# careylab/LocoMouse_cpp

Measured on AMD Instinct MI355X. Metric: frames/sec whole-node + achieved HBM GB/s; 1024×256 gray, 6 templates, higher is better.
Workload: dtype f32

## Files before the change

### include/locomouse_hip.h

```cpp
#ifndef LOCOMOUSE_HIP_H
#define LOCOMOUSE_HIP_H

#include <stddef.h>
#include <stdint.h>

#ifdef __cplusplus
extern "C" {
#endif

#define LM_ABI_VERSION 6
#define LM_N_PAWS 4
#define LM_N_TAIL_POINTS 15
#define LM_N_LISTS 4
#define LM_N_FEATURES 2

typedef enum {
  LM_OK = 0,
  LM_ERR_INVALID_ARGUMENT = 1,
  LM_ERR_RUNTIME = 2,
  LM_ERR_HIP = 3
} lm_status;

typedef struct {
  int32_t x, y, width, height;
// ... 145 lines not shown

lm_status lm_ctx_set_debug(lm_ctx* ctx, int32_t flags);

lm_status lm_debug_scores(lm_ctx* ctx, int32_t f, int32_t det, float* out, int32_t rows, int32_t cols);

lm_status lm_debug_tail_mask(lm_ctx* ctx, int32_t f, uint8_t* out, int32_t rows, int32_t cols);

int32_t lm_debug_kernel_times(lm_ctx* ctx, const char** names, double* ms, int32_t cap);

int32_t lm_debug_kernel_spans(lm_ctx* ctx, const char** names, double* t0, double* t1, int32_t cap);

lm_status lm_debug_corr_work(const lm_ctx* ctx, int32_t* out);

lm_status lm_debug_tail_work(lm_ctx* ctx, int32_t* out);

lm_status lm_debug_tail_tiles(lm_ctx* ctx, int32_t f, int32_t view, uint8_t* out, int32_t rows, int32_t cols);

lm_status lm_debug_point_work(lm_ctx* ctx, int32_t* out);

lm_status lm_debug_point_tiles(lm_ctx* ctx, int32_t f, int32_t det, uint8_t* out, int32_t rows, int32_t cols);

int32_t lm_debug_dark_tile_width(void);
int32_t lm_debug_dark_tile_height(void);

int32_t lm_debug_batch_slots(const lm_ctx* ctx);


#define LM_BB_FIRSTLAST_AS_EXECUTED 0
#define LM_BB_FIRSTLAST_INTEGER 1

// ... 53 lines not shown
```

### locomouse_cpp_amd/csrc/lm_device.h

```cpp
#ifndef LM_DEVICE_H
#define LM_DEVICE_H

#include <stdint.h>

#if defined(__HIPCC__)
#define LM_HD __host__ __device__
#else
#define LM_HD
#endif

#define LM_C 5
#define LM_R 3
#define LM_TW (16 * LM_C)
#define LM_TH (16 * LM_R)
#define LM_JC 4
#ifndef LM_FW
#define LM_FW 40
#endif
#ifndef LM_FH
#define LM_FH 4
#endif
static_assert((LM_FW == 40 || LM_FW == 80) && (LM_FH == 4 || LM_FH == 8), "dark-tile grid");
#define LM_RW_NQX (LM_TW / LM_FW)
#define LM_RW_NQY (16 / LM_FH)
// ... 47 lines not shown
  int32_t tail_w, tail_hb, tail_hs;
  int32_t tail_cap, tail_ntc;
  int32_t tail_nw, tail_bm_words;
  int32_t connectivity;
  int32_t fl_tx[2], fl_ty[2], fl_off[2], fl_slot;
  int32_t tl_stride;
  int32_t tt_tx[2], tt_ty[2], tt_off[2], tt_slot;
  int32_t tt_stride;
  int64_t pt_plane;
  int32_t tb_skip[LM_NDET], tb_off[LM_NDET], tb_rng[LM_NDET], tb_lds[2];
  double tb_bias[LM_NDET];
  int32_t tbw_br[2], tbw_nband[2], tbw_blo[2], tbw_nbk[2], tbw_rows[2], tbw_v[2], tbw_al[2], tbw_work[2], tbw_lds[2];
  int32_t tbw_use[LM_NDET], tbw_pn[LM_NDET], tbw_win[LM_NDET], tbw_wsz[LM_NDET], tbw_ent[LM_NDET];
  uint32_t tbw_inv[LM_NDET];
  int32_t tbr_on[LM_NDET], tbr_ng[LM_NDET], tbr_off[LM_NDET];
  int32_t fl_my[2], fl_mx[2], fl_oh[2], fl_ow[2];
  int32_t ing_b0[2], ing_nb[2], ing_threads;
  int32_t list_cap[LM_NLIST];
  int64_t list_off[LM_NLIST];
  int64_t keys_per_slot;
  double side_bottom_min_overlap;
  double alpha_vel_bottom, pairwise_occluded_cost;
  int32_t max_displacement_bottom, ong_spacing_bottom;
  int32_t ong_nx, ong_ny;
  double ong_br_x, ong_br_y;
  int32_t bb_bottom_w, bb_bottom_h;
  int32_t spre_b_w, spre_b_h, spre_t_w, spre_t_h;
  int32_t match_b[LM_NFEAT][4];
  int32_t match_s[LM_NFEAT][4];
  int32_t size_b[LM_NFEAT][2];
// ... 108 lines not shown
```

### locomouse_cpp_amd/csrc/lm_kernels.hip

```cpp
#include <hip/hip_runtime.h>
#include <stdint.h>

#include <type_traits>
#include <utility>

#include "lm_device.h"
#include "lm_introsort.h"

#include "lm_dev_common.h"
#include "lm_tail_bound.h"
#include "lm_tile_plan.h"



__global__ __launch_bounds__(LM_MM_THREADS) void k_minmax(const uint8_t* const* __restrict__ frame_ptr,
                                                          const uint8_t* __restrict__ bkg, int npix, int s0,
                                                          unsigned* __restrict__ mm) {
  const int slot = s0 + blockIdx.y;
  const lm_gu8* __restrict__ F = as_global(frame_ptr[slot]);
  const int nvec = npix >> 4;
  const int per = (nvec + LM_MM_SPLIT - 1) / LM_MM_SPLIT;
  const int v0 = blockIdx.x * per, v1 = min(nvec, v0 + per);
  const lm_gu4* F4 = reinterpret_cast<const lm_gu4*>(F);
  const uint4* B4 = reinterpret_cast<const uint4*>(bkg);
// ... 626 lines not shown
  if (m == 0ull) return 0;
  const int rank = (int)__builtin_amdgcn_mbcnt_hi((unsigned)(m >> 32), __builtin_amdgcn_mbcnt_lo((unsigned)m, 0u));
  int base = 0;
  if (p && rank == 0) base = atomicAdd(ctr, (int)__popcll(m));
  return __shfl(base, __ffsll((long long)m) - 1) + rank;
}
#ifndef LM_TBW_WPE
#define LM_TBW_WPE 8
#endif
#define TBW_SEL(a) (k == 0 ? a[0] : k == 1 ? a[1] : a[2])
template <bool ROWS>
__global__ __launch_bounds__(LM_TB_THREADS) __attribute__((amdgpu_waves_per_eu(LM_TBW_WPE, 8))) void k_tile_bound(
    const LmConst* __restrict__ Kp, const uint32_t* __restrict__ rng, int64_t rng_slot, int s0, int nslot,
    const double* __restrict__ tbc, const uint8_t* __restrict__ bright, uint8_t* __restrict__ tail_flags,
    int32_t* __restrict__ tt_cnt, uint32_t* __restrict__ tt_list, uint8_t* __restrict__ pt_flags,
    int32_t* __restrict__ pt_cnt, uint32_t* __restrict__ pt_list) {
  const LmConst& K = *Kp;
  extern __shared__ __attribute__((aligned(16))) uint8_t tbw_lds[];
  __shared__ int s_n[3], s_b[3], s_m[3], s_base[3], s_nw;
  const int v = (int)blockIdx.y < K.tbw_nband[0] ? 0 : 1;
  const int band = (int)blockIdx.y - (v ? K.tbw_nband[0] : 0);
  const int slot = s0 + (int)blockIdx.x;
  const int T = (int)blockDim.x, tid = (int)threadIdx.x;
  if (tid < 3) {
    s_n[tid] = 0;
    s_b[tid] = 0;
    s_m[tid] = 0;
  }
  if (tid == 0) s_nw = 0;
  bool on[3], use[3], refine[3], tail[3];
  int t0[3], nt[3], ohb[3], ftx[3], tbase[3];
// ... 207 lines not shown
    constexpr int WV = 64;
    const int c1 = (nr3[0] * LM_TB_NBX + WV - 1) / WV, c2 = c1 + (nr3[1] * LM_TB_NBX + WV - 1) / WV,
              c3 = c2 + (nr3[2] * LM_TB_NBX + WV - 1) / WV;
    const uint32_t rcx = lm_rcp(LM_TB_NBX);
    for (int ch = __builtin_amdgcn_readfirstlane(tid / WV); ch < c3; ch += T / WV) {
      const int k = ch < c1 ? 0 : ch < c2 ? 1 : 2;
      const int d = 3 * v + k;
      const LmDet& D = K.det[d];
      const int n = TBW_SEL(nr3), fx = TBW_SEL(ftx), tk0 = TBW_SEL(t0), ohk = TBW_SEL(ohb);
      const int e = (ch - (k == 0 ? 0 : k == 1 ? c1 : c2)) * WV + (tid & (WV - 1));
      const int mb = k == 0 ? 0 : k == 1 ? nr3[0] : nr3[0] + nr3[1];
      const uint32_t* ent = reinterpret_cast<const uint32_t*>(tbw_lds + K.tbw_ent[d]);
      const int kh = D.kh, ng = K.tbr_ng[d], nc = lm_tbr_chunks(ng);
      const double* __restrict__ C = tbc + K.tbr_off[d];
      const double bias = K.tb_bias[d];
      const int yb = D.in_y + LM_FH * tk0 - y_lo;
      const int bl0 = lm_tbr_block0(D.in_x, 0) - K.tbw_blo[v];
      const int bendl = lm_tbr_block_end(D.in_x, D.ow, D.kw, K.ext_w[v] / LM_TB_BLK) - K.tbw_blo[v];
      const int nbx = (D.ow + LM_TB_BLK - 1) / LM_TB_BLK;
      if (e >= n * LM_TB_NBX) continue;
      const int t = lm_div(e, rcx);
      const int tile = (int)(ent[t] & 0xFFFFu);
      const int ty = lm_div(tile, K.tbw_inv[d]), tx = tile - ty * fx;
      const int xb = tx * LM_TB_NBX + (e - t * LM_TB_NBX);
      if (xb >= nbx) continue;
      const int tyb = ty - tk0;
      const int nr = min(LM_TB_H, ohk - LM_TB_H * tyb);
      const int row0 = yb + LM_TB_H * tyb, ba0 = bl0 + xb;
      auto level_v = [&](auto rows) {
        const uint32_t* pw = V + row0 * nw + (ba0 >> 1);
        const uint16_t* alone = AL + k * als + row0;
        const bool clipped = ba0 + ng == bendl;
        const int jl = (ng - 1) % LM_TBR_GC;
        uint32_t w0, w1, w2, x0 = 0u, x1 = 0u;
        unsigned qn, q = 0u;
        bool lastc = false;
        auto fetch = [&]() {
          w0 = pw[0];
          w1 = pw[1];
          w2 = pw[2];
          qn = *alone;
        };
        fetch();
        if constexpr (decltype(rows)::value > 0) {
          constexpr int NG = decltype(rows)::value;
          return lm_tbr_sum_rows_n<NG>(kh, C, bias, [&](int i, int g, unsigned& M, unsigned& m) {
                   if (g == 0) {
                     lm_tbr_quad_align(w0, w1, w2, ba0, x0, x1);
                     q = qn;
                     pw += nw;
                     alone += 1;
                     fetch();
                   }
                   lm_tbr_quad_get(x0, x1, g, g == NG - 1 && clipped, q, M, m);
                 }) < 0.0;
        }
        return lm_tbr_sum_negative(kh, ng, C, bias, [&](int i, int g, unsigned& M, unsigned& m) {
          if (g % LM_TBR_GC == 0) {
            const int c = g / LM_TBR_GC;
            lm_tbr_quad_align(w0, w1, w2, ba0, x0, x1);
            q = qn;
            lastc = c == nc - 1;
            pw += lastc ? nw - 2 * (nc - 1) : 2;
            alone += lastc ? 1 : 0;
            fetch();
          }
          lm_tbr_quad_get(x0, x1, g % LM_TBR_GC, lastc && clipped && g % LM_TBR_GC == jl, q, M, m);
        });
      };
      auto level_b = [&](int rs, int nn) {
        return lm_tbr_sum_negative(kh, ng, C, bias, [&](int i, int g, unsigned& M, unsigned& m) {
          const uint16_t* row = B16 + (row0 + rs + i) * nbk;
          M = 0u;
          m = 255u;
          for (int r = 0; r < nn; ++r, row += nbk) {
            unsigned a, b;
            lm_tbr_pair_range(nullptr, row, ba0 + g, bendl, a, b);
            M = max(M, a);
            m = min(m, b);
          }
        });
      };
      using std::integral_constant;
      bool proven;
      if constexpr (!ROWS) {
        proven = nr == LM_TB_H && level_v(integral_constant<int, 0>{});
      } else {
        proven = false;
        if (nr != LM_TB_H) {
        } else if (nc != 1) proven = level_v(integral_constant<int, 0>{});
        else if (ng == 4) proven = level_v(integral_constant<int, 4>{});
        else if (ng == 3) proven = level_v(integral_constant<int, 3>{});
        else if (ng == 2) proven = level_v(integral_constant<int, 2>{});
        else proven = level_v(integral_constant<int, 1>{});
      }
      if (!proven && !(LM_TB_RH == LM_TB_H && nr == LM_TB_H)) {
        if (LM_TB_RH == LM_TB_H) {
          proven = level_b(0, nr);
        } else {
          proven = true;
          for (int r = 0; r < nr && proven; ++r) proven = level_b(r, 1);
        }
      }
      if (!proven) mark[mb + t] = 1u;
    }
    __syncthreads();
    constexpr int CR = LM_TBW_CR;
    for (int g0 = 0; g0 < nref; g0 += CR * T) {
      uint32_t en[CR];
// ... 1848 lines not shown
```

### locomouse_cpp_amd/csrc/lm_runtime.hip

```cpp
#include <hip/hip_runtime.h>

#include <algorithm>
#include <array>
#include <cmath>
#include <cstdio>
#include <cstring>
#include <map>
#include <numeric>
#include <atomic>
#include <deque>
#include <memory>
#include <mutex>
#include <stdexcept>
#include <string>
#include <thread>
#include <vector>

#include "locomouse_hip.h"
#include "lm_host.h"
#include "lm_kernels.hip"

namespace {

constexpr size_t kCorrLdsBudget = 64 * 1024;
// ... 153 lines not shown
  } corr_plan[2];
  DevBuf<uint8_t> bkg, adj;
  DevBuf<int32_t> cal;
  DevBuf<float> weights;
  DevBuf<_Float16> weights16;
  DevBuf<LmConst> dK;
  size_t tail_lds = 0;
  bool tail_big = false;
  int64_t tail_ws_slot = 0;
  bool kprof_on = false;
  bool dark_on = true;
  bool tailskip_on = true;
  bool pointskip_on = true;
  bool tb_ref = false;
  bool tb_refine = true;
  bool corr_dir_on = true;
  size_t tb_lds = 0;
  size_t tbw_lds = 0;
  bool tbw_row_loop = false;
  DevBuf<double> tb_const;
  std::vector<std::unique_ptr<Lane>> lanes;
  DevBuf<uint8_t> handoff;
  std::vector<std::unique_ptr<HostBuf<uint8_t>>> packs;
  std::vector<char> pack_busy;
  int take_pack(size_t cap) {
    size_t i = 0;
    while (i < packs.size() && pack_busy[i]) ++i;
    if (i == packs.size()) {
      packs.emplace_back(new HostBuf<uint8_t>());
      pack_busy.push_back(0);
    }
    if (packs[i]->n < cap) packs[i]->alloc(cap);
    pack_busy[i] = 1;
    return (int)i;
  }
// ... 101 lines not shown
        (f16_nch(dets[d]->cols) > LM_F16_MAX_NCH || f16_lds_bytes(f16_nch(dets[d]->cols), dets[d]->rows) > kF16LdsMax))
      throw std::invalid_argument(std::string(names[d]) + ": detector too large for the f16 correlation (LM_CORR_F16).");
  }
  if (su->corr_precision != LM_CORR_FP32 && su->corr_precision != LM_CORR_F16)
    throw std::invalid_argument("corr_precision must be LM_CORR_FP32 or LM_CORR_F16.");
}

LmTileSwitches read_switches(lm_ctx* c, const lm_setup* su) {
  auto flag = [](const char* name, bool dflt) {
    const char* v = getenv(name);
    return v ? atoi(v) != 0 : dflt;
  };
  c->kprof_on = flag("LM_KPROF", false);
  c->dark_on = flag("LM_CORR_DARK", true);
  c->tb_refine = flag("LM_TILE_REFINE", true);
  c->tb_ref = flag("LM_TILE_BOUND_REF", false);
  c->corr_dir_on = flag("LM_CORR_DIR", true);
  LmTileSwitches sw;
  sw.tailskip = flag("LM_CORR_TAILSKIP", true);
  sw.pointskip = flag("LM_CORR_POINTSKIP", true);
  sw.refine = c->tb_refine;
  sw.f16 = su->corr_precision == LM_CORR_F16;
  sw.dark = c->dark_on;
  return sw;
}

lm_geometry make_geometry(const lm_setup* su, const lm_params* P, const lm_model* M) {
  const int NR = su->calib_rows, NC = su->calib_cols;
  const lm_rect ub = P->bounding_box_bottom, us = P->bounding_box_side;
  lm_geometry g;
  std::memset(&g, 0, sizeof(g));
  g.n_rows = NR;
  g.n_cols = NC;
  const int mts_c = std::max(M->paw_side.cols, M->snout_side.cols), mts_r = std::max(M->paw_side.rows, M->snout_side.rows);
  const int mtb_c = std::max(M->paw_bottom.cols, M->snout_bottom.cols), mtb_r = std::max(M->paw_bottom.rows, M->snout_bottom.rows);
  g.spre_t_w = ceil_half(mts_c - 1);
// ... 371 lines not shown
  const int64_t nc = (int64_t)su->calib_rows * su->calib_cols;
  hipStream_t cs = nullptr;
  HIPCHK(hipStreamCreateWithFlags(&cs, hipStreamNonBlocking));
  struct StreamGuard {
    hipStream_t s;
    ~StreamGuard() { (void)hipStreamDestroy(s); }
  } cs_guard{cs};
  c->bkg.alloc(nv);
  COPY_SYNC(c->bkg.p, su->background, nv, hipMemcpyHostToDevice, cs);
  c->cal.alloc(nc);
  COPY_SYNC(c->cal.p, su->ind_warp_mapping, nc * sizeof(int32_t), hipMemcpyHostToDevice, cs);
  c->weights.alloc(wts.size());
  COPY_SYNC(c->weights.p, wts.data(), wts.size() * sizeof(float), hipMemcpyHostToDevice, cs);
  c->tb_const.alloc(tbc.size());
  COPY_SYNC(c->tb_const.p, tbc.data(), tbc.size() * sizeof(double), hipMemcpyHostToDevice, cs);
  if (!w16.empty()) {
    c->weights16.alloc(w16.size());
    COPY_SYNC(c->weights16.p, w16.data(), w16.size() * sizeof(_Float16), hipMemcpyHostToDevice, cs);
  }
  c->adj.alloc(256);
  COPY_SYNC(c->adj.p, adj, 256, hipMemcpyHostToDevice, cs);
  c->dK.alloc(1);
  COPY_SYNC(c->dK.p, &c->K, sizeof(LmConst), hipMemcpyHostToDevice, cs);
  c->fstride = (nv + 255) / 256 * 256;
  HIPCHK(hipFuncSetAttribute((const void*)k_tail<false>, hipFuncAttributeMaxDynamicSharedMemorySize, (int)c->tail_lds));
  HIPCHK(hipFuncSetAttribute((const void*)k_tile_bound_ref, hipFuncAttributeMaxDynamicSharedMemorySize, (int)c->tb_lds));
  HIPCHK(hipFuncSetAttribute((const void*)k_tile_bound<false>, hipFuncAttributeMaxDynamicSharedMemorySize, (int)c->tbw_lds));
  HIPCHK(hipFuncSetAttribute((const void*)k_tile_bound<true>, hipFuncAttributeMaxDynamicSharedMemorySize, (int)c->tbw_lds));
  for (const auto& P : c->corr_plan)
    for (size_t g = 0; g < P.groups.size(); ++g)
// ... 409 lines not shown
    k_ingest<<<dim3((unsigned)(K.ing_nb[0] + K.ing_nb[1]), (unsigned)((nproc + LM_INGEST_FB - 1) / LM_INGEST_FB)),
               K.ing_threads, 0, st>>>(dK, L.frame_ptr.p, c->bkg.p, c->cal.p, L.luts.p, L.slots.p, s_proc0, n + 1, L.ext.p,
                                        c->ext_slot_bytes, reinterpret_cast<unsigned*>(L.tailbin.p), L.smap.p, L.sbkg.p,
                                        L.skey.p, dk.flags, dk.cnt, dk.list, L.rng.p, kpi);
    T.end();
    if (dk.tail_cnt || dk.pt_cnt) {
      T.begin("k_tile_bound");
      if (c->tb_ref)
        k_tile_bound_ref<<<dim3((unsigned)nproc, 2), LM_TB_THREADS, c->tb_lds, st>>>(
            dK, L.ext.p, c->ext_slot_bytes, s_proc0, c->tb_const.p, dk.flags, dk.tail_flags, dk.tail_cnt, dk.tail_list,
            dk.pt_flags, dk.pt_cnt, dk.pt_list);
      else
        (c->tbw_row_loop ? k_tile_bound<true> : k_tile_bound<false>)
            <<<dim3((unsigned)nproc, (unsigned)(K.tbw_nband[0] + K.tbw_nband[1])), LM_TB_THREADS, c->tbw_lds, st>>>(
                dK, L.rng.p, c->ext_slot_bytes / LM_INGEST_VEC, s_proc0, nproc, c->tb_const.p, dk.flags, dk.tail_flags,
                dk.tail_cnt, dk.tail_list, dk.pt_flags, dk.pt_cnt, dk.pt_list);
      T.end();
    }
    const lm_ctx::CorrPlan& CP = c->corr_plan[P.plan];
    if (c->corr_dir_on && std::find(CP.ring.begin(), CP.ring.end(), (char)1) != CP.ring.end()) {
      std::vector<LmDetGroup> groups;
      for (const auto& grp : CP.groups) groups.push_back(grp.second);
      HIPCHK(launch_corr_dir(st, dK, groups.data(), CP.ring.data(), (int)groups.size(), nproc, dk, L.corr_dir.p,
                             L.err.p));
    }
  }
  if (part == 1 || part < 0) {
    T.begin("k_corr");
    const lm_ctx::CorrPlan& CP = c->corr_plan[P.plan];
    for (size_t gi = 0; gi < CP.groups.size(); ++gi) {
      const auto& grp = CP.groups[gi];
// ... 674 lines not shown
  if (!ctx->tailskip_on) return LM_OK;
  const Lane* Lp = delivered_lane(ctx);
  if (!Lp) return fail(LM_ERR_INVALID_ARGUMENT, kLaneReused);
  const Lane& L = *Lp;
  return guarded([&] {
    HIPCHK(hipSetDevice(ctx->device));
    int32_t h[2 * LM_TL_NC];
    COPY_SYNC(h, L.tail_cnt.p, sizeof(h), hipMemcpyDeviceToHost, L.stream);
    for (int t = 0; t < 2; ++t) {
      out[2 * t] = std::accumulate(h + t * LM_TL_NC, h + (t + 1) * LM_TL_NC, 0);
      out[2 * t + 1] = ctx->delivered.slots * ctx->K.tt_tx[t] * ctx->K.tt_ty[t];
    }
  });
}

LM_API lm_status lm_debug_tail_tiles(lm_ctx* ctx, int32_t f, int32_t view, uint8_t* out, int32_t rows, int32_t cols) {
  if (!ctx || !out) return fail(LM_ERR_INVALID_ARGUMENT, "null argument");
  if (!ctx->tailskip_on) return fail(LM_ERR_INVALID_ARGUMENT, "tail-tile skipping is off");
  const Lane* Lp = delivered_lane(ctx);
  if (!Lp) return fail(LM_ERR_INVALID_ARGUMENT, kLaneReused);
  const Lane& L = *Lp;
  if (f < 0 || f >= L.batch_n || view < 0 || view > 1) return fail(LM_ERR_INVALID_ARGUMENT, "index out of range");
  if (rows != ctx->K.tt_ty[view] || cols != ctx->K.tt_tx[view]) return fail(LM_ERR_INVALID_ARGUMENT, "shape mismatch");
  return guarded([&] {
    HIPCHK(hipSetDevice(ctx->device));
    COPY_SYNC(out, L.tail_flags.p + (int64_t)(f + 1) * ctx->K.tt_slot + ctx->K.tt_off[view], (size_t)rows * cols,
              hipMemcpyDeviceToHost, L.stream);
  });
}

// ... 129 lines not shown
```

### locomouse_cpp_amd/csrc/lm_tail_bound.h

```cpp
#ifndef LM_TAIL_BOUND_H
#define LM_TAIL_BOUND_H

#include <stdint.h>

#if defined(__HIPCC__)
#define LM_TB_HD __host__ __device__
#else
#define LM_TB_HD
#endif

#define LM_TB_W 40
#define LM_TB_H 4
#define LM_TB_BLK 8

LM_TB_HD inline int lm_tb_prepare(const float* w, int kh, int kw, int wstride, float delta, double* P, double* N,
                                  double* bias) {
  int ok = 1;
  double sabs = 0.0;
  for (int i = 0; i < kh; ++i) {
    double p = 0.0, n = 0.0;
    for (int j = 0; j < kw; ++j) {
      const double v = (double)w[i * wstride + j];
      if (!(v - v == 0.0)) ok = 0;
      if (v > 0.0) p += v;
// ... 214 lines not shown
}
template <class F>
LM_TB_HD inline double lm_tbr_sum_rows(int kh, int ng, const double* C, double bias, F&& rng) {
  switch (ng) {
    case 1: return lm_tbr_sum_rows_n<1>(kh, C, bias, rng);
    case 2: return lm_tbr_sum_rows_n<2>(kh, C, bias, rng);
    case 3: return lm_tbr_sum_rows_n<3>(kh, C, bias, rng);
    case 4: return lm_tbr_sum_rows_n<4>(kh, C, bias, rng);
    default: return lm_tbr_sum(kh, ng, C, bias, rng);
  }
}
template <class F>
LM_TB_HD inline bool lm_tbr_sum_negative(int kh, int ng, const double* C, double bias, F&& rng) {
  return lm_tbr_sum(kh, ng, C, bias, rng) < 0.0;
}
LM_TB_HD inline int lm_tbr_block0(int in_x, int xb) { return in_x / LM_TB_BLK + xb; }
LM_TB_HD inline int lm_tbr_block_end(int in_x, int ow, int kw, int nbw) {
  const int e = (in_x + ow + kw - 1 + LM_TB_BLK - 1) / LM_TB_BLK;
  return e < nbw ? e : nbw;
}
LM_TB_HD inline bool lm_tbr_block_skip(const uint8_t* bmax, const uint8_t* bmin, int nbw, int in_y, int in_x, int ow,
                                       int kh, int kw, int y, int nr, int xb, const double* C, double bias) {
  const int b0 = lm_tbr_block0(in_x, xb), bend = lm_tbr_block_end(in_x, ow, kw, nbw);
  return lm_tbr_sum_negative(kh, lm_tbr_groups(in_x, kw), C, bias, [&](int i, int g, unsigned& M, unsigned& m) {
    const int ba = b0 + g, bb = ba + 1 < bend ? ba + 1 : bend - 1;
    M = 0u;
    m = 255u;
    for (int r = 0; r < nr; ++r) {
      const int row = (in_y + y + i + r) * nbw;
      const unsigned xa = bmax[row + ba], xb2 = bmax[row + bb], na = bmin[row + ba], nb = bmin[row + bb];
      M = xa > M ? xa : M;
      M = xb2 > M ? xb2 : M;
      m = na < m ? na : m;
      m = nb < m ? nb : m;
    }
  });
}
LM_TB_HD inline uint32_t lm_tb_range_merge(uint32_t a, uint32_t b) {
  const uint32_t a0 = a & 0xFFu, b0 = b & 0xFFu, a1 = a & 0xFF00u, b1 = b & 0xFF00u;
  const uint32_t a2 = a & 0xFF0000u, b2 = b & 0xFF0000u, a3 = a & 0xFF000000u, b3 = b & 0xFF000000u;
  return (a0 > b0 ? a0 : b0) | (a1 < b1 ? a1 : b1) | (a2 > b2 ? a2 : b2) | (a3 < b3 ? a3 : b3);
}
LM_TB_HD inline uint32_t lm_tbr_pair_word(uint32_t w, uint32_t wnext, bool last) {
  return lm_tb_range_merge(w, (w >> 16) | (last ? w & 0xFFFF0000u : wnext << 16));
}
LM_TB_HD inline void lm_tbr_pair_range(const uint16_t* pair, const uint16_t* plain, int ba, int bendl, unsigned& M,
                                       unsigned& m) {
  if (pair != nullptr) {
    const unsigned q = ba == bendl - 1 ? plain[ba] : pair[ba];
    M = q & 0xFFu;
    m = q >> 8;
  } else {
// ... 39 lines not shown
```

### locomouse_cpp_amd/csrc/lm_tile_plan.h

```cpp
#ifndef LM_TILE_PLAN_H
#define LM_TILE_PLAN_H

#include <stdint.h>

#include <algorithm>
#include <stdexcept>
#include <vector>

#include "lm_device.h"
#include "lm_tail_bound.h"

#define LM_INGEST_VEC 16
static_assert(LM_FW >= LM_INGEST_VEC, "a 16-byte chunk spans at most two flag tiles");
static_assert(LM_TB_BLK == 8 && LM_INGEST_VEC == 2 * LM_TB_BLK, "a 16-byte chunk holds two blocks");
#define LM_INGEST_MAXTX 128

static_assert(LM_TB_W == LM_FW && LM_TB_H == LM_FH, "the bound's tiles are the dark-tile grid's");
#define LM_TB_THREADS 256
#ifndef LM_TBW_TILES
#define LM_TBW_TILES LM_TB_THREADS
#endif
#ifndef LM_TBW_ROW_LOOP
#define LM_TBW_ROW_LOOP 1
#endif

constexpr int64_t kTbRefLds = 144 * 1024;
constexpr int64_t kTbwLds = 64 * 1024;

struct LmTileSwitches {
  bool tailskip;
  bool pointskip;
  bool refine;
  bool f16;
  bool dark;
};

struct LmTilePlan {
  std::vector<double> tbc;
  size_t tb_lds = 0;
  size_t tbw_lds = 0;
  bool row_loop = false;
  bool tailskip = false, pointskip = false;
};

struct LmTbwView {
  int v;
  int ftx[3], ty[3];
  bool on[3];
  int sum_tx;
// ... 13 lines not shown
    const LmDet& D = K.det[t ? DET_TAIL_S : DET_TAIL_B];
    K.tt_tx[t] = (D.ow + LM_FW - 1) / LM_FW;
    K.tt_ty[t] = (D.oh + LM_FH - 1) / LM_FH;
    K.tt_off[t] = o;
    o += (K.tt_tx[t] * K.tt_ty[t] + 3) / 4 * 4;
    mt = std::max(mt, K.tt_tx[t] * K.tt_ty[t]);
  }
  K.tt_slot = o;
  K.tt_stride = nslots * mt;
  if (mt > 65535 || nslots > 65535) *tailskip = false;
  static_assert(LIST_PAW_B == 0 && LIST_SNOUT_B == 1 && LIST_PAW_S == 2 && LIST_SNOUT_S == 3, "list l: feature l & 1");
  K.pt_plane = (int64_t)K.fl_slot * nslots;
  if (K.fl_tx[0] * K.fl_ty[0] > 65535 || K.fl_tx[1] * K.fl_ty[1] > 65535 || nslots > 65535) *pointskip = false;
}

inline void lm_tp_bounds(LmConst& K, int v, const float* wts, bool tailskip, bool pointskip, bool refine,
                         std::vector<double>& tbc) {
  int64_t lds = 2 * (int64_t)K.ext_h[v] * (K.ext_w[v] / LM_TB_BLK);
  bool any = false;
  for (int d : {3 * v + 2, 3 * v, 3 * v + 1}) {
    const LmDet& D = K.det[d];
    K.tb_off[d] = (int32_t)tbc.size();
    tbc.resize(tbc.size() + 2 * (size_t)D.kh);
    K.tb_skip[d] = lm_tb_prepare(wts + D.w_off, D.kh, D.kw, D.kwp, D.delta, tbc.data() + K.tb_off[d],
                                 tbc.data() + K.tb_off[d] + D.kh, &K.tb_bias[d]);
    const int64_t rows = (int64_t)D.oh + D.kh - 1, wcols = (int64_t)D.ow + D.kw - 1;
    const int64_t need = 2 * rows * (D.kind != 0 ? K.tt_tx[v] : K.fl_tx[v]);
    const bool inside = D.in_y >= 0 && D.in_x >= 0 && D.in_y + rows <= K.ext_h[v] && D.in_x + wcols <= K.ext_w[v];
    if (!(D.kind != 0 ? tailskip : pointskip) || !inside || lds + need > kTbRefLds) K.tb_skip[d] = 0;
    K.tb_rng[d] = K.tb_skip[d] ? (int32_t)lds : 0;
    if (K.tb_skip[d]) {
      lds += need;
      any = true;
    }
    K.tbr_on[d] = K.tb_skip[d] && refine ? 1 : 0;
    K.tbr_ng[d] = K.tbr_on[d] ? lm_tbr_groups(D.in_x, D.kw) : 0;
    tbc.resize((tbc.size() + 7) / 8 * 8);
    K.tbr_off[d] = (int32_t)tbc.size();
    if (K.tbr_on[d]) {
      tbc.resize(tbc.size() + (size_t)lm_tbr_const_size(D.kh, K.tbr_ng[d]));
      lm_tbr_prepare(wts + D.w_off, D.kh, D.kw, D.kwp, D.in_x, tbc.data() + K.tbr_off[d]);
    }
  }
  K.tb_lds[v] = any ? (int32_t)lds : 0;
}

inline LmTbwView lm_tbw_view(const LmConst& K, int v, bool tailskip, bool pointskip) {
  LmTbwView W{};
  W.v = v;
  int max_ty = 1;
  for (int k = 0; k < 3; ++k) {
    const LmDet& D = K.det[3 * v + k];
    W.ftx[k] = D.kind != 0 ? K.tt_tx[v] : K.fl_tx[v];
    W.ty[k] = D.kind != 0 ? K.tt_ty[v] : K.fl_ty[v];
    W.on[k] = D.kind != 0 ? tailskip : pointskip;
    if (W.on[k]) {
      W.sum_tx += W.ftx[k];
// ... 107 lines not shown
    K.tbw_pn[d] = L.pn[k];
    K.tbw_win[d] = L.win[k];
    K.tbw_wsz[d] = L.wsz[k];
    K.tbw_ent[d] = L.ent[k];
  }
}

inline LmTilePlan lm_tile_plan(LmConst& K, int nslots, const float* wts, const LmTileSwitches& sw) {
  LmTilePlan R;
  R.tailskip = sw.tailskip;
  R.pointskip = sw.pointskip;
  if (sw.f16) R.tailskip = R.pointskip = false;
  if (!sw.dark) R.pointskip = false;
  lm_tp_grids(K, nslots, &R.tailskip, &R.pointskip);
  for (int v = 0; v < 2; ++v) {
    lm_tp_bounds(K, v, wts, R.tailskip, R.pointskip, sw.refine, R.tbc);
    R.tb_lds = std::max(R.tb_lds, (size_t)K.tb_lds[v]);
  }
  for (int v = 0; v < 2; ++v) {
    lm_tp_bands(K, v, R.tailskip, R.pointskip);
    R.tbw_lds = std::max(R.tbw_lds, (size_t)K.tbw_lds[v]);
  }
  bool one_chunk = false;
  for (int d = 0; d < LM_NDET; ++d)
    one_chunk = one_chunk || (K.tbw_use[d] && K.tbr_on[d] && lm_tbr_chunks(K.tbr_ng[d]) == 1);
  R.row_loop = LM_TBW_ROW_LOOP && one_chunk;
  return R;
}

#endif
```

### locomouse_cpp_amd/runtime.py

```python
import ctypes as C
import os
import subprocess

import numpy as np

from .abi import (BB_FRAME_DTYPE, LM_ENC_GRAY8, LM_ENC_RGB24, LM_OK, lm_batch_result, lm_bb_result, lm_enc_mark,
                  lm_enc_overlay, lm_enc_result, lm_enc_stats, lm_geometry, lm_jpeg_info, lm_jpeg_interval_stats, lm_jpeg_stats,
                  lm_train_point, lm_train_stats, result_to_numpy)

PKG = os.path.dirname(os.path.abspath(__file__))
ROOT = os.path.dirname(PKG)
LIB_PATH = os.path.join(PKG, "liblocomouse_hip.so")
CSRC = os.path.join(PKG, "csrc")

EXPORTED = (
    "lm_abi_version", "lm_last_error", "lm_ctx_create", "lm_ctx_destroy", "lm_get_geometry", "lm_ctx_stream",
    "lm_detect_batch", "lm_detect_batch_device", "lm_ctx_set_debug", "lm_debug_scores", "lm_debug_tail_mask",
    "lm_debug_kernel_times", "lm_debug_kernel_spans", "lm_synth_frames_device",
    "lm_bb_create", "lm_bb_destroy", "lm_bb_push", "lm_bb_push_device", "lm_bb_finish", "lm_bb_debug_binary",
    "lm_bb_stream", "lm_host_alloc", "lm_host_free",
    "lm_detect_submit", "lm_detect_submit_device", "lm_detect_collect", "lm_ctx_lanes", "lm_ctx_pending",
    "lm_debug_corr_work", "lm_debug_batch_slots", "lm_debug_dark_tile_width",
    "lm_debug_dark_tile_height", "lm_debug_tail_work", "lm_debug_tail_tiles", "lm_debug_point_work",
    "lm_debug_point_tiles",
)

HIPCC_FLAGS = ["--offload-arch=gfx950", "-O3", "-std=c++17", "-fPIC", "-shared", "-ffp-contract=off", "-fno-slp-vectorize",
               "-fvisibility=hidden", "-Wall", "-Wno-unused-function", "-Wno-unused-variable"]


HOST_DIR = os.path.join(PKG, "host")
HOST_LIB_PATH = os.path.join(PKG, "liblocomouse_host.so")
CLI_PATH = os.path.join(PKG, "bin", "LocoMouse")


HIP_UNITS = ("lm_runtime.hip", "lm_corr.hip", "lm_bbox.hip", "lm_jpeg.hip", "lm_bkg.hip", "lm_jpeg_enc.hip",
             "lm_train.hip")

JPEG_EXPORTED = ("lm_jpeg_create", "lm_jpeg_destroy", "lm_jpeg_decode_device", "lm_jpeg_probe", "lm_jpeg_stream",
# ... 123 lines not shown
            fn.argtypes = [C.c_void_p]
            fn.restype = C.c_int32
        L.lm_ctx_set_debug.argtypes = [C.c_void_p, C.c_int32]
        L.lm_debug_scores.argtypes = [C.c_void_p, C.c_int32, C.c_int32, C.c_void_p, C.c_int32, C.c_int32]
        L.lm_debug_tail_mask.argtypes = [C.c_void_p, C.c_int32, C.c_void_p, C.c_int32, C.c_int32]
        L.lm_debug_kernel_times.argtypes = [C.c_void_p, C.POINTER(C.c_char_p), C.POINTER(C.c_double), C.c_int32]
        L.lm_debug_kernel_times.restype = C.c_int32
        L.lm_debug_kernel_spans.argtypes = [C.c_void_p, C.POINTER(C.c_char_p), C.POINTER(C.c_double),
                                            C.POINTER(C.c_double), C.c_int32]
        L.lm_debug_kernel_spans.restype = C.c_int32
        L.lm_debug_corr_work.argtypes = [C.c_void_p, C.POINTER(C.c_int32)]
        L.lm_debug_tail_work.argtypes = [C.c_void_p, C.POINTER(C.c_int32)]
        L.lm_debug_tail_tiles.argtypes = [C.c_void_p, C.c_int32, C.c_int32, C.c_void_p, C.c_int32, C.c_int32]
        L.lm_debug_point_work.argtypes = [C.c_void_p, C.POINTER(C.c_int32)]
        L.lm_debug_point_tiles.argtypes = [C.c_void_p, C.c_int32, C.c_int32, C.c_void_p, C.c_int32, C.c_int32]
        L.lm_debug_batch_slots.argtypes = [C.c_void_p]
        L.lm_debug_batch_slots.restype = C.c_int32
        L.lm_synth_frames_device.argtypes = [C.c_int32, C.c_void_p, C.c_int32, C.c_int32, C.c_int64, C.c_int32,
                                             C.c_int64]
        L.lm_bb_create.argtypes = [C.c_int32, C.c_void_p, C.c_void_p, C.c_int32, C.POINTER(C.c_void_p)]
        L.lm_bb_destroy.argtypes = [C.c_void_p]
        for fn in (L.lm_bb_push, L.lm_bb_push_device):
            fn.argtypes = [C.c_void_p, C.c_void_p, C.c_int64, C.c_int32, C.c_void_p]
        L.lm_bb_finish.argtypes = [C.c_void_p, C.POINTER(lm_bb_result)]
        L.lm_bb_debug_binary.argtypes = [C.c_void_p, C.c_int32, C.c_void_p, C.c_int32, C.c_int32]
        L.lm_host_alloc.argtypes = [C.c_size_t, C.POINTER(C.c_void_p)]
        L.lm_host_free.argtypes = [C.c_void_p]
        L.lm_bb_stream.argtypes = [C.c_void_p]
        L.lm_bb_stream.restype = C.c_void_p
        L.lm_jpeg_create.argtypes = [C.c_int32, C.c_int32, C.c_int32, C.c_int32, C.c_int32, C.POINTER(C.c_void_p)]
# ... 177 lines not shown
        t0 = (C.c_double * 64)()
        t1 = (C.c_double * 64)()
        n = lib().lm_debug_kernel_spans(self._h, names, t0, t1, 64)
        return [(names[i].decode(), t0[i], t1[i]) for i in range(min(n, 64))]

    def corr_work(self):
        out = (C.c_int32 * 4)()
        _check(lib().lm_debug_corr_work(self._h, out))
        return None if out[0] < 0 else {"tiles": (out[0], out[1]), "outputs": (out[2], out[3])}

    def tail_work(self):
        out = (C.c_int32 * 4)()
        _check(lib().lm_debug_tail_work(self._h, out))
        return None if out[0] < 0 else {"listed": (out[0], out[2]), "total": (out[1], out[3])}

    def tail_tiles(self, f, view):
        g = self.geometry()
        tw, th = self.dark_tile_shape()
        oh = (g.bb_side_mouse if view else g.bb_bottom_mouse).height
        out = np.zeros((-(-oh // th), -(-g.tail_box_width // tw)), dtype=np.uint8)
        _check(lib().lm_debug_tail_tiles(self._h, f, view, out.ctypes.data, out.shape[0], out.shape[1]))
        return out

    def point_work(self):
        out = (C.c_int32 * 8)()
        _check(lib().lm_debug_point_work(self._h, out))
        return None if out[0] < 0 else {"listed": tuple(out[0:8:2]), "bright": tuple(out[1:8:2])}

    def point_tiles(self, f, det):
        g = self.geometry()
# ... 365 lines not shown
```

Before: 939,200.

## Screen tile bounds with fp32 sums and a rigorous error margin before the fp64 path

Adds an fp32 screening pass to the single-chunk tile-bound test in k_tile_bound. Constants are rounded outward to float and a proven error bound E is computed on the host. The kernel first evaluates the bound with packed fp32 FMAs and decides the tile only when the sum clears ±E, falling back to the existing fp64 sum otherwise. This is meant to cut fp64 arithmetic cost in the tile-skip kernel. It adds a per-wave atomic counter of fallbacks, a second evaluation for undecided tiles, and extra constant storage.

```diff
diff --git a/include/locomouse_hip.h b/include/locomouse_hip.h
--- a/include/locomouse_hip.h
+++ b/include/locomouse_hip.h
@@ -183,6 +183,8 @@
 
 lm_status lm_debug_tail_work(lm_ctx* ctx, int32_t* out);
 
+lm_status lm_debug_screen_fallback(lm_ctx* ctx, int64_t* out);
+
 lm_status lm_debug_tail_tiles(lm_ctx* ctx, int32_t f, int32_t view, uint8_t* out, int32_t rows, int32_t cols);
 
 lm_status lm_debug_point_work(lm_ctx* ctx, int32_t* out);
diff --git a/locomouse_cpp_amd/csrc/lm_device.h b/locomouse_cpp_amd/csrc/lm_device.h
--- a/locomouse_cpp_amd/csrc/lm_device.h
+++ b/locomouse_cpp_amd/csrc/lm_device.h
@@ -85,6 +85,8 @@
   int32_t tbw_use[LM_NDET], tbw_pn[LM_NDET], tbw_win[LM_NDET], tbw_wsz[LM_NDET], tbw_ent[LM_NDET];
   uint32_t tbw_inv[LM_NDET];
   int32_t tbr_on[LM_NDET], tbr_ng[LM_NDET], tbr_off[LM_NDET];
+  int32_t tbs_on[LM_NDET], tbs_off[LM_NDET];
+  float tbs_bf[LM_NDET], tbs_e[LM_NDET];
   int32_t fl_my[2], fl_mx[2], fl_oh[2], fl_ow[2];
   int32_t ing_b0[2], ing_nb[2], ing_threads;
   int32_t list_cap[LM_NLIST];
diff --git a/locomouse_cpp_amd/csrc/lm_kernels.hip b/locomouse_cpp_amd/csrc/lm_kernels.hip
--- a/locomouse_cpp_amd/csrc/lm_kernels.hip
+++ b/locomouse_cpp_amd/csrc/lm_kernels.hip
@@ -664,7 +664,7 @@
     const LmConst* __restrict__ Kp, const uint32_t* __restrict__ rng, int64_t rng_slot, int s0, int nslot,
     const double* __restrict__ tbc, const uint8_t* __restrict__ bright, uint8_t* __restrict__ tail_flags,
     int32_t* __restrict__ tt_cnt, uint32_t* __restrict__ tt_list, uint8_t* __restrict__ pt_flags,
-    int32_t* __restrict__ pt_cnt, uint32_t* __restrict__ pt_list) {
+    int32_t* __restrict__ pt_cnt, uint32_t* __restrict__ pt_list, unsigned long long* __restrict__ tbs_fallback) {
   const LmConst& K = *Kp;
   extern __shared__ __attribute__((aligned(16))) uint8_t tbw_lds[];
   __shared__ int s_n[3], s_b[3], s_m[3], s_base[3], s_nw;
@@ -902,6 +902,7 @@
       const int kh = D.kh, ng = K.tbr_ng[d], nc = lm_tbr_chunks(ng);
       const double* __restrict__ C = tbc + K.tbr_off[d];
       const double bias = K.tb_bias[d];
+      const float* __restrict__ Cf = reinterpret_cast<const float*>(tbc + K.tbs_off[d]);
       const int yb = D.in_y + LM_FH * tk0 - y_lo;
       const int bl0 = lm_tbr_block0(D.in_x, 0) - K.tbw_blo[v];
       const int bendl = lm_tbr_block_end(D.in_x, D.ow, D.kw, K.ext_w[v] / LM_TB_BLK) - K.tbw_blo[v];
@@ -915,7 +916,7 @@
       const int tyb = ty - tk0;
       const int nr = min(LM_TB_H, ohk - LM_TB_H * tyb);
       const int row0 = yb + LM_TB_H * tyb, ba0 = bl0 + xb;
-      auto level_v = [&](auto rows) {
+      auto level_v = [&](auto rows, auto screen) {
         const uint32_t* pw = V + row0 * nw + (ba0 >> 1);
         const uint16_t* alone = AL + k * als + row0;
         const bool clipped = ba0 + ng == bendl;
@@ -932,16 +933,20 @@
         fetch();
         if constexpr (decltype(rows)::value > 0) {
           constexpr int NG = decltype(rows)::value;
-          return lm_tbr_sum_rows_n<NG>(kh, C, bias, [&](int i, int g, unsigned& M, unsigned& m) {
-                   if (g == 0) {
-                     lm_tbr_quad_align(w0, w1, w2, ba0, x0, x1);
-                     q = qn;
-                     pw += nw;
-                     alone += 1;
-                     fetch();
-                   }
-                   lm_tbr_quad_get(x0, x1, g, g == NG - 1 && clipped, q, M, m);
-                 }) < 0.0;
+          auto term = [&](int i, int g, unsigned& M, unsigned& m) {
+            if (g == 0) {
+              lm_tbr_quad_align(w0, w1, w2, ba0, x0, x1);
+              q = qn;
+              pw += nw;
+              alone += 1;
+              fetch();
+            }
+            lm_tbr_quad_get(x0, x1, g, g == NG - 1 && clipped, q, M, m);
+          };
+          if constexpr (decltype(screen)::value)
+            return lm_tbs_decide(lm_tbs_sum_rows_n<NG>(kh, Cf, K.tbs_bf[d], term), K.tbs_e[d]);
+          else
+            return lm_tbr_sum_rows_n<NG>(kh, C, bias, term) < 0.0 ? -1 : 1;
         }
         return lm_tbr_sum_negative(kh, ng, C, bias, [&](int i, int g, unsigned& M, unsigned& m) {
           if (g % LM_TBR_GC == 0) {
@@ -954,7 +959,7 @@
             fetch();
           }
           lm_tbr_quad_get(x0, x1, g % LM_TBR_GC, lastc && clipped && g % LM_TBR_GC == jl, q, M, m);
-        });
+        }) ? -1 : 1;
       };
       auto level_b = [&](int rs, int nn) {
         return lm_tbr_sum_negative(kh, ng, C, bias, [&](int i, int g, unsigned& M, unsigned& m) {
@@ -970,17 +975,34 @@
         });
       };
       using std::integral_constant;
+      using std::false_type;
+      using std::true_type;
       bool proven;
       if constexpr (!ROWS) {
-        proven = nr == LM_TB_H && level_v(integral_constant<int, 0>{});
+        proven = nr == LM_TB_H && level_v(integral_constant<int, 0>{}, false_type{}) < 0;
       } else {
         proven = false;
         if (nr != LM_TB_H) {
-        } else if (nc != 1) proven = level_v(integral_constant<int, 0>{});
-        else if (ng == 4) proven = level_v(integral_constant<int, 4>{});
-        else if (ng == 3) proven = level_v(integral_constant<int, 3>{});
-        else if (ng == 2) proven = level_v(integral_constant<int, 2>{});
-        else proven = level_v(integral_constant<int, 1>{});
+        } else if (nc != 1) proven = level_v(integral_constant<int, 0>{}, false_type{}) < 0;
+        else {
+          int dec = 0;
+          if (K.tbs_on[d] != 0) {
+            if (ng == 4) dec = level_v(integral_constant<int, 4>{}, true_type{});
+            else if (ng == 3) dec = level_v(integral_constant<int, 3>{}, true_type{});
+            else if (ng == 2) dec = level_v(integral_constant<int, 2>{}, true_type{});
+            else dec = level_v(integral_constant<int, 1>{}, true_type{});
+            const unsigned long long und = __ballot(dec == 0);
+            if (und != 0ull && (tid & (WV - 1)) == __ffsll((long long)und) - 1)
+              atomicAdd(tbs_fallback, (unsigned long long)__popcll(und));
+          }
+          if (dec == 0) {
+            if (ng == 4) dec = level_v(integral_constant<int, 4>{}, false_type{});
+            else if (ng == 3) dec = level_v(integral_constant<int, 3>{}, false_type{});
+            else if (ng == 2) dec = level_v(integral_constant<int, 2>{}, false_type{});
+            else dec = level_v(integral_constant<int, 1>{}, false_type{});
+          }
+          proven = dec < 0;
+        }
       }
       if (!proven && !(LM_TB_RH == LM_TB_H && nr == LM_TB_H)) {
         if (LM_TB_RH == LM_TB_H) {
diff --git a/locomouse_cpp_amd/csrc/lm_runtime.hip b/locomouse_cpp_amd/csrc/lm_runtime.hip
--- a/locomouse_cpp_amd/csrc/lm_runtime.hip
+++ b/locomouse_cpp_amd/csrc/lm_runtime.hip
@@ -191,11 +191,13 @@
   bool pointskip_on = true;
   bool tb_ref = false;
   bool tb_refine = true;
+  bool tb_screen = true;
   bool corr_dir_on = true;
   size_t tb_lds = 0;
   size_t tbw_lds = 0;
   bool tbw_row_loop = false;
   DevBuf<double> tb_const;
+  DevBuf<unsigned long long> tbs_fallback;
   std::vector<std::unique_ptr<Lane>> lanes;
   DevBuf<uint8_t> handoff;
   std::vector<std::unique_ptr<HostBuf<uint8_t>>> packs;
@@ -327,12 +329,14 @@
   c->kprof_on = flag("LM_KPROF", false);
   c->dark_on = flag("LM_CORR_DARK", true);
   c->tb_refine = flag("LM_TILE_REFINE", true);
+  c->tb_screen = flag("LM_TILE_SCREEN", true);
   c->tb_ref = flag("LM_TILE_BOUND_REF", false);
   c->corr_dir_on = flag("LM_CORR_DIR", true);
   LmTileSwitches sw;
   sw.tailskip = flag("LM_CORR_TAILSKIP", true);
   sw.pointskip = flag("LM_CORR_POINTSKIP", true);
   sw.refine = c->tb_refine;
+  sw.screen = c->tb_screen;
   sw.f16 = su->corr_precision == LM_CORR_F16;
   sw.dark = c->dark_on;
   return sw;
@@ -734,6 +738,8 @@
   COPY_SYNC(c->weights.p, wts.data(), wts.size() * sizeof(float), hipMemcpyHostToDevice, cs);
   c->tb_const.alloc(tbc.size());
   COPY_SYNC(c->tb_const.p, tbc.data(), tbc.size() * sizeof(double), hipMemcpyHostToDevice, cs);
+  c->tbs_fallback.alloc(1);
+  SET_SYNC(c->tbs_fallback.p, 0, sizeof(unsigned long long), cs);
   if (!w16.empty()) {
     c->weights16.alloc(w16.size());
     COPY_SYNC(c->weights16.p, w16.data(), w16.size() * sizeof(_Float16), hipMemcpyHostToDevice, cs);
@@ -1173,7 +1179,7 @@
         (c->tbw_row_loop ? k_tile_bound<true> : k_tile_bound<false>)
             <<<dim3((unsigned)nproc, (unsigned)(K.tbw_nband[0] + K.tbw_nband[1])), LM_TB_THREADS, c->tbw_lds, st>>>(
                 dK, L.rng.p, c->ext_slot_bytes / LM_INGEST_VEC, s_proc0, nproc, c->tb_const.p, dk.flags, dk.tail_flags,
-                dk.tail_cnt, dk.tail_list, dk.pt_flags, dk.pt_cnt, dk.pt_list);
+                dk.tail_cnt, dk.tail_list, dk.pt_flags, dk.pt_cnt, dk.pt_list, c->tbs_fallback.p);
       T.end();
     }
     const lm_ctx::CorrPlan& CP = c->corr_plan[P.plan];
@@ -1878,6 +1884,19 @@
   });
 }
 
+LM_API lm_status lm_debug_screen_fallback(lm_ctx* ctx, int64_t* out) {
+  if (!ctx || !out) return fail(LM_ERR_INVALID_ARGUMENT, "null argument");
+  *out = 0;
+  if (ctx->lanes.empty() || !ctx->tbs_fallback.p) return LM_OK;
+  return guarded([&] {
+    HIPCHK(hipSetDevice(ctx->device));
+    for (const auto& L : ctx->lanes) HIPCHK(hipStreamSynchronize(L->stream));
+    unsigned long long h = 0;
+    COPY_SYNC(&h, ctx->tbs_fallback.p, sizeof(h), hipMemcpyDeviceToHost, ctx->lanes[0]->stream);
+    *out = (int64_t)h;
+  });
+}
+
 LM_API lm_status lm_debug_tail_tiles(lm_ctx* ctx, int32_t f, int32_t view, uint8_t* out, int32_t rows, int32_t cols) {
   if (!ctx || !out) return fail(LM_ERR_INVALID_ARGUMENT, "null argument");
   if (!ctx->tailskip_on) return fail(LM_ERR_INVALID_ARGUMENT, "tail-tile skipping is off");
diff --git a/locomouse_cpp_amd/csrc/lm_tail_bound.h b/locomouse_cpp_amd/csrc/lm_tail_bound.h
--- a/locomouse_cpp_amd/csrc/lm_tail_bound.h
+++ b/locomouse_cpp_amd/csrc/lm_tail_bound.h
@@ -1,6 +1,7 @@
 #ifndef LM_TAIL_BOUND_H
 #define LM_TAIL_BOUND_H
 
+#include <math.h>
 #include <stdint.h>
 
 #if defined(__HIPCC__)
@@ -252,6 +253,111 @@
 LM_TB_HD inline bool lm_tbr_sum_negative(int kh, int ng, const double* C, double bias, F&& rng) {
   return lm_tbr_sum(kh, ng, C, bias, rng) < 0.0;
 }
+#define LM_TBS_ROW (2 * LM_TBR_GC)
+struct LmTbsConst {
+  float bf, E;
+  int on;
+};
+inline float lm_tbs_up(double x) {
+  float f = (float)x;
+  return (double)f < x ? nextafterf(f, INFINITY) : f;
+}
+inline float lm_tbs_down(double x) { return -lm_tbs_up(-x); }
+inline LmTbsConst lm_tbs_prepare(const double* C, int kh, int ng, double bias, int ok, float* Cf) {
+  LmTbsConst R;
+  R.on = ok && ng >= 1 && ng <= LM_TBR_GC ? 1 : 0;
+  const double tiny = 1.17549435082228750797e-38;
+  double sum = 0.0;
+  for (int i = 0; i < kh; ++i)
+    for (int g = 0; g < LM_TBR_GC; ++g) {
+      const double p = g < ng && R.on ? C[i * 2 * LM_TBR_GC + g] : 0.0, n = g < ng && R.on ? C[(i * 2 + 1) * LM_TBR_GC + g] : 0.0;
+      if (!(p - p == 0.0) || !(n - n == 0.0) || (p != 0.0 && p < tiny) || (n != 0.0 && n < tiny) || p > 1e30 || n > 1e30) {
+        R.on = 0;
+        Cf[i * LM_TBS_ROW + 2 * g] = Cf[i * LM_TBS_ROW + 2 * g + 1] = 0.f;
+        continue;
+      }
+      const float pf = lm_tbs_up(p), nf = lm_tbs_down(n);
+      Cf[i * LM_TBS_ROW + 2 * g] = pf;
+      Cf[i * LM_TBS_ROW + 2 * g + 1] = -nf;
+      sum += (double)pf + (double)nf;
+    }
+  const double ab = bias < 0.0 ? -bias : bias;
+  if (!(bias - bias == 0.0) || (bias != 0.0 && ab < tiny) || ab > 1e30) {
+    R.on = 0;
+    R.bf = 0.f;
+  } else {
+    R.bf = lm_tbs_up(bias);
+  }
+  const double n = (double)kh * (double)ng, af = R.bf < 0.f ? -(double)R.bf : (double)R.bf;
+  const double S = af + 255.0 * sum;
+  const double E = (2.0 * (2.0 * n + 4.0) / 16777216.0 + 1e-12 + (n + 2.0) / 2251799813685248.0) * S + (n + 1.0) * 2.4e-38;
+  if (!(S < 1e30) || !(n < 1048576.0)) R.on = 0;
+  R.E = R.on ? lm_tbs_up(E) : 0.f;
+  return R;
+}
+#if defined(__clang__)
+typedef float lm_tbs_f2 __attribute__((ext_vector_type(2)));
+LM_TB_HD inline lm_tbs_f2 lm_tbs_fma2(float x0, float x1, float c0, float c1, lm_tbs_f2 acc) {
+  return __builtin_elementwise_fma(lm_tbs_f2{x0, x1}, lm_tbs_f2{c0, c1}, acc);
+}
+#else
+struct lm_tbs_f2 {
+  float x, y;
+};
+inline lm_tbs_f2 lm_tbs_fma2(float x0, float x1, float c0, float c1, lm_tbs_f2 acc) {
+  return lm_tbs_f2{fmaf(x0, c0, acc.x), fmaf(x1, c1, acc.y)};
+}
+#endif
+template <int NG, class F>
+LM_TB_HD inline float lm_tbs_sum_rows_n(int kh, const float* Cf, float bf, F&& rng) {
+  static_assert(LM_TBR_GC == 4 && NG >= 1 && NG <= LM_TBR_GC, "a row is read as four pairs");
+  lm_tbs_f2 acc = {bf, 0.f};
+  auto row = [&](int i, float c0, float c1, float c2, float c3, float c4, float c5, float c6, float c7, auto&& ahead) {
+    unsigned M, m;
+    rng(i, 0, M, m);
+    ahead();
+    acc = lm_tbs_fma2((float)M, (float)m, c0, c1, acc);
+    if (NG > 1) {
+      rng(i, 1, M, m);
+      acc = lm_tbs_fma2((float)M, (float)m, c2, c3, acc);
+    }
+    if (NG > 2) {
+      rng(i, 2, M, m);
+      acc = lm_tbs_fma2((float)M, (float)m, c4, c5, acc);
+    }
+    if (NG > 3) {
+      rng(i, 3, M, m);
+      acc = lm_tbs_fma2((float)M, (float)m, c6, c7, acc);
+    }
+  };
+  if (kh > 0) {
+    const float* q = Cf;
+    float a0 = q[0], a1 = q[1], a2 = q[2], a3 = q[3], a4 = q[4], a5 = q[5], a6 = q[6], a7 = q[7];
+    float b0 = 0.f, b1 = 0.f, b2 = 0.f, b3 = 0.f, b4 = 0.f, b5 = 0.f, b6 = 0.f, b7 = 0.f;
+    for (int i = 0; i < kh; i += 2, q += 2 * LM_TBS_ROW) {
+      const float* qb = q + (i + 1 < kh ? LM_TBS_ROW : 0);
+      row(i, a0, a1, a2, a3, a4, a5, a6, a7,
+          [&] { b0 = qb[0], b1 = qb[1], b2 = qb[2], b3 = qb[3], b4 = qb[4], b5 = qb[5], b6 = qb[6], b7 = qb[7]; });
+      if (i + 1 < kh) {
+        const float* qa = qb + (i + 2 < kh ? LM_TBS_ROW : 0);
+        row(i + 1, b0, b1, b2, b3, b4, b5, b6, b7,
+            [&] { a0 = qa[0], a1 = qa[1], a2 = qa[2], a3 = qa[3], a4 = qa[4], a5 = qa[5], a6 = qa[6], a7 = qa[7]; });
+      }
+    }
+  }
+  return acc.x + acc.y;
+}
+template <class F>
+LM_TB_HD inline float lm_tbs_sum_rows(int kh, int ng, const float* Cf, float bf, F&& rng) {
+  switch (ng) {
+    case 1: return lm_tbs_sum_rows_n<1>(kh, Cf, bf, rng);
+    case 2: return lm_tbs_sum_rows_n<2>(kh, Cf, bf, rng);
+    case 3: return lm_tbs_sum_rows_n<3>(kh, Cf, bf, rng);
+    default: return lm_tbs_sum_rows_n<4>(kh, Cf, bf, rng);
+  }
+}
+LM_TB_HD inline int lm_tbs_decide(float Uf, float E) { return Uf < -E ? -1 : Uf >= E ? 1 : 0; }
+
 LM_TB_HD inline int lm_tbr_block0(int in_x, int xb) { return in_x / LM_TB_BLK + xb; }
 LM_TB_HD inline int lm_tbr_block_end(int in_x, int ow, int kw, int nbw) {
   const int e = (in_x + ow + kw - 1 + LM_TB_BLK - 1) / LM_TB_BLK;
@@ -274,6 +380,24 @@
     }
   });
 }
+LM_TB_HD inline int lm_tbs_block(const uint8_t* bmax, const uint8_t* bmin, int nbw, int in_y, int in_x, int ow, int kh,
+                                 int kw, int y, int nr, int xb, const float* Cf, float bf, float E) {
+  const int b0 = lm_tbr_block0(in_x, xb), bend = lm_tbr_block_end(in_x, ow, kw, nbw);
+  const float Uf = lm_tbs_sum_rows(kh, lm_tbr_groups(in_x, kw), Cf, bf, [&](int i, int g, unsigned& M, unsigned& m) {
+    const int ba = b0 + g, bb = ba + 1 < bend ? ba + 1 : bend - 1;
+    M = 0u;
+    m = 255u;
+    for (int r = 0; r < nr; ++r) {
+      const int row = (in_y + y + i + r) * nbw;
+      const unsigned xa = bmax[row + ba], xb2 = bmax[row + bb], na = bmin[row + ba], nb = bmin[row + bb];
+      M = xa > M ? xa : M;
+      M = xb2 > M ? xb2 : M;
+      m = na < m ? na : m;
+      m = nb < m ? nb : m;
+    }
+  });
+  return lm_tbs_decide(Uf, E);
+}
 LM_TB_HD inline uint32_t lm_tb_range_merge(uint32_t a, uint32_t b) {
   const uint32_t a0 = a & 0xFFu, b0 = b & 0xFFu, a1 = a & 0xFF00u, b1 = b & 0xFF00u;
   const uint32_t a2 = a & 0xFF0000u, b2 = b & 0xFF0000u, a3 = a & 0xFF000000u, b3 = b & 0xFF000000u;
diff --git a/locomouse_cpp_amd/csrc/lm_tile_plan.h b/locomouse_cpp_amd/csrc/lm_tile_plan.h
--- a/locomouse_cpp_amd/csrc/lm_tile_plan.h
+++ b/locomouse_cpp_amd/csrc/lm_tile_plan.h
@@ -4,6 +4,7 @@
 #include <stdint.h>
 
 #include <algorithm>
+#include <cstring>
 #include <stdexcept>
 #include <vector>
 
@@ -33,6 +34,7 @@
   bool refine;
   bool f16;
   bool dark;
+  bool screen = true;
 };
 
 struct LmTilePlan {
@@ -76,7 +78,7 @@
   if (K.fl_tx[0] * K.fl_ty[0] > 65535 || K.fl_tx[1] * K.fl_ty[1] > 65535 || nslots > 65535) *pointskip = false;
 }
 
-inline void lm_tp_bounds(LmConst& K, int v, const float* wts, bool tailskip, bool pointskip, bool refine,
+inline void lm_tp_bounds(LmConst& K, int v, const float* wts, bool tailskip, bool pointskip, bool refine, bool screen,
                          std::vector<double>& tbc) {
   int64_t lds = 2 * (int64_t)K.ext_h[v] * (K.ext_w[v] / LM_TB_BLK);
   bool any = false;
@@ -103,6 +105,19 @@
       tbc.resize(tbc.size() + (size_t)lm_tbr_const_size(D.kh, K.tbr_ng[d]));
       lm_tbr_prepare(wts + D.w_off, D.kh, D.kw, D.kwp, D.in_x, tbc.data() + K.tbr_off[d]);
     }
+    K.tbs_on[d] = 0;
+    K.tbs_off[d] = (int32_t)tbc.size();
+    K.tbs_bf[d] = K.tbs_e[d] = 0.f;
+    if (K.tbr_on[d] && screen && lm_tbr_chunks(K.tbr_ng[d]) == 1) {
+      static_assert(LM_TBS_ROW * sizeof(float) == 4 * sizeof(double), "a row of the screen's floats is four doubles");
+      std::vector<float> cf((size_t)D.kh * LM_TBS_ROW);
+      const LmTbsConst R = lm_tbs_prepare(tbc.data() + K.tbr_off[d], D.kh, K.tbr_ng[d], K.tb_bias[d], 1, cf.data());
+      tbc.resize(tbc.size() + cf.size() / 2);
+      std::memcpy(tbc.data() + K.tbs_off[d], cf.data(), cf.size() * sizeof(float));
+      K.tbs_on[d] = R.on;
+      K.tbs_bf[d] = R.bf;
+      K.tbs_e[d] = R.E;
+    }
   }
   K.tb_lds[v] = any ? (int32_t)lds : 0;
 }
@@ -240,7 +255,7 @@
   if (!sw.dark) R.pointskip = false;
   lm_tp_grids(K, nslots, &R.tailskip, &R.pointskip);
   for (int v = 0; v < 2; ++v) {
-    lm_tp_bounds(K, v, wts, R.tailskip, R.pointskip, sw.refine, R.tbc);
+    lm_tp_bounds(K, v, wts, R.tailskip, R.pointskip, sw.refine, sw.screen, R.tbc);
     R.tb_lds = std::max(R.tb_lds, (size_t)K.tb_lds[v]);
   }
   for (int v = 0; v < 2; ++v) {
diff --git a/locomouse_cpp_amd/runtime.py b/locomouse_cpp_amd/runtime.py
--- a/locomouse_cpp_amd/runtime.py
+++ b/locomouse_cpp_amd/runtime.py
@@ -22,7 +22,7 @@
     "lm_detect_submit", "lm_detect_submit_device", "lm_detect_collect", "lm_ctx_lanes", "lm_ctx_pending",
     "lm_debug_corr_work", "lm_debug_batch_slots", "lm_debug_dark_tile_width",
     "lm_debug_dark_tile_height", "lm_debug_tail_work", "lm_debug_tail_tiles", "lm_debug_point_work",
-    "lm_debug_point_tiles",
+    "lm_debug_point_tiles", "lm_debug_screen_fallback",
 )
 
 HIPCC_FLAGS = ["--offload-arch=gfx950", "-O3", "-std=c++17", "-fPIC", "-shared", "-ffp-contract=off", "-fno-slp-vectorize",
@@ -176,6 +176,7 @@
         L.lm_debug_tail_tiles.argtypes = [C.c_void_p, C.c_int32, C.c_int32, C.c_void_p, C.c_int32, C.c_int32]
         L.lm_debug_point_work.argtypes = [C.c_void_p, C.POINTER(C.c_int32)]
         L.lm_debug_point_tiles.argtypes = [C.c_void_p, C.c_int32, C.c_int32, C.c_void_p, C.c_int32, C.c_int32]
+        L.lm_debug_screen_fallback.argtypes = [C.c_void_p, C.POINTER(C.c_int64)]
         L.lm_debug_batch_slots.argtypes = [C.c_void_p]
         L.lm_debug_batch_slots.restype = C.c_int32
         L.lm_synth_frames_device.argtypes = [C.c_int32, C.c_void_p, C.c_int32, C.c_int32, C.c_int64, C.c_int32,
@@ -383,6 +384,11 @@
         _check(lib().lm_debug_tail_work(self._h, out))
         return None if out[0] < 0 else {"listed": (out[0], out[2]), "total": (out[1], out[3])}
 
+    def screen_fallback(self):
+        out = C.c_int64(0)
+        _check(lib().lm_debug_screen_fallback(self._h, C.byref(out)))
+        return int(out.value)
+
     def tail_tiles(self, f, view):
         g = self.geometry()
         tw, th = self.dark_tile_shape()
```

New measurement: 960,900 (median of 6 runs). 1.02x the previous value.
